# mjrgh/DCSExplorer

Hardware: AMD Instinct MI355X
Metric: bit_exact_int16_pcm_samples_per_sec (higher is better)
Workload: dtype int16; 1 GPU; survey3_65536; gpu_max_hw_queues=4, samples_per_frame=240, frames_per_wave=8, wavefronts_per_launch=8192, arithmetic=ADSP-2105 1.15 fixed point, 32-bit integer intermediates, partition=range over streams, no collective, scale=1, inflight=1, frames_per_chunk=all, full=False

## Files before the change

### dcsexplorer_amd/csrc/dcs_decode_chunk.inc.h

```cpp
    DCS_STAMP(1);

    struct { uint32_t job; uint32_t prevSlot, flags, nSrc, shiftXform; uint32_t firstSrc, prevJob, poolOff, bpl; } slot;
    uint32_t exportNext;
    uint4 pd0, pd1, phdr;
    uint2 pd2;
    uint32_t planHdr0 = 0, planHdr1 = 0, planType0 = 0, planType1 = 0;
    {
        uint4 *scratch = reinterpret_cast<uint4 *>(L.pool());
        static_assert(kHeadVec * 16 <= poolDwords(FPW) * 4, "the package head fits in the bit pool");
        if (lane < kHeadVec)
            scratch[lane] = phead0;
        if (kHeadLoads > 1 && lane + 64 < kHeadVec)
            scratch[lane + 64] = phead1;
        waveSync();
        const uint4 *sp5 = scratch + 5 * s;
        const uint4 s0 = sp5[0];
        pd0 = sp5[1]; pd1 = sp5[2];
        const uint4 d2v = sp5[3];
        pd2 = make_uint2(d2v.x, d2v.y);
        phdr = sp5[4];
        if constexpr (bandPlanInLds(FPW))
        {
            const unsigned char *bytes = reinterpret_cast<const unsigned char *>(sp5) + q;
            planType0 = bytes[36]; planType1 = bytes[44];
            planHdr0 = bytes[64]; planHdr1 = bytes[72];
        }
        waveSync();
        slot.job = s0.x;
        slot.prevSlot = s0.y & 0xFFu; slot.flags = (s0.y >> 8) & 0xFFu; slot.nSrc = (s0.y >> 16) & 0xFFu; slot.shiftXform = s0.y >> 24;
        slot.firstSrc = s0.z; slot.prevJob = s0.w;
        slot.poolOff = d2v.z & 0xFFFFu;
        slot.bpl = (d2v.z >> 16) & 0xFFu;
        const unsigned long long exportSlots = __ballot(lane < FPW && !(slot.flags & DCS_SLOT_EMPTY) && (slot.flags & DCS_SLOT_EXPORT) != 0);
        exportNext = static_cast<uint32_t>(__builtin_amdgcn_readlane(static_cast<int>(d2v.w), exportSlots != 0 ? static_cast<int>(__builtin_ctzll(exportSlots)) : 0));
    }

    if constexpr (bandPlanInLds(FPW))
    {
        const int fmt0 = static_cast<int>((pd0.z >> 16) & 0xFFu);
        if (__any(!(slot.flags & DCS_SLOT_EMPTY) && slot.nSrc != 0 && fmt0 >= DCS_FMT_94_T0))
        {
            uint2 *plan = reinterpret_cast<uint2 *>(L.plan());
            const uint2 *tmpl = reinterpret_cast<const uint2 *>(smem + planTableOffset(FPW));
            const bool type1 = fmt0 != DCS_FMT_94_T0;
            const uint32_t keyLim = type1 ? 16u : 17u;
            const uint32_t cls0 = !type1 ? DCS_B94_TYPE0 : q < 3 ? 0u : q < 6 ? 17u : 34u, cls1 = type1 ? 34u : DCS_B94_TYPE0;
            const uint32_t pre = (type1 && q < 3) ? (pd2.y >> (4 * q)) & 15u : 0u;
            plan[lane] = planBand94(L.tables(), tmpl, planHdr0, planType0, cls0, keyLim, q < 2 ? 7u + q : 16u, pre);
            plan[lane + 64] = planBand94(L.tables(), tmpl, planHdr1, planType1, cls1, keyLim, q == 7 ? 32u : 16u, 0u);
        }
    }

    const int firstXform = __builtin_amdgcn_readfirstlane(static_cast<int>(slot.shiftXform >> 4)) == DCS_XFORM_94 ? DCS_XFORM_94 : DCS_XFORM_93;
    if (PASS == 0 || firstXform != constsXform)
    {
        constsXform = firstXform;
        loadLaneConsts(a.tables, lane, constsXform, C);
    }
#pragma unroll
    for (int t = 0 ; t < kPoolPieces ; ++t)
    {
        const int i = lane * 4 + 256 * t;
        const bool in = i < imgDw;
        if (i < poolDwords(FPW))
            ldsWrite4(L.pool() + i, in ? pimg[t].x : 0u, in ? pimg[t].y : 0u, in ? pimg[t].z : 0u, in ? pimg[t].w : 0u);
    }

    const bool live = !(slot.flags & DCS_SLOT_EMPTY);
    struct { uint32_t firstSrc; int nSrc; int volShift; int xform; uint32_t prev; } job;
    job.firstSrc = slot.firstSrc; job.nSrc = slot.nSrc; job.volShift = slot.shiftXform & 15;
    job.xform = slot.shiftXform >> 4; job.prev = slot.prevJob;

    uint32_t err = 0;
    {
        uint32_t *pool = L.pool();
        const DcsLdsTables *T = L.tables();
        uint16_t *row = L.row(s);
        const uint32_t *blobW = reinterpret_cast<const uint32_t *>(a.blob);
        const uint32_t blobWords = static_cast<uint32_t>((a.blobLen + 3) >> 2);
        const int myNSrc = live ? job.nSrc : 0;

        auto unpackRound = [&](auto r0tag, const int r)
        {
            constexpr bool R0 = decltype(r0tag)::value;
            const bool has = r < myNSrc;
            const uint4 *sdp = reinterpret_cast<const uint4 *>(&a.srcs[has ? job.firstSrc + r : 0]);
            uint4 d0 = make_uint4(0, 0, 0, 0), d1 = d0;
            uint2 d2 = make_uint2(0, 0);
            uint2 sp = make_uint2(0, 0);
            const int bplSlot = slot.bpl;
            if (R0)
            {
                if (has) { d0 = pd0; d1 = pd1; d2 = pd2; sp = psplit; }
            }
            else if (has) { d0 = sdp[0]; d1 = sdp[1]; d2 = *reinterpret_cast<const uint2 *>(sdp + 2); }
            const uint64_t streamOff = static_cast<uint64_t>(d0.x) | (static_cast<uint64_t>(d0.y) << 32);
            const uint32_t mixMul = d0.z & 0xFFFFu;
            const int format = static_cast<int>((d0.z >> 16) & 0xFFu);
            const int hdrLen = has ? static_cast<int>(d0.z >> 24) : 16;
            const uint32_t bitOff = d0.w;
            const uint32_t nBits = d1.x & 0xFFFFu, hdrBits = d1.x >> 16;
            const int nBands = static_cast<int>((d2.y >> 16) & 0xFFu);
            const uint32_t flags = d2.y >> 24;
            const bool serial = R0 ? bplSlot == 0 : ((flags & DCS_IDX_SERIAL) != 0 || SUB == 1);

            Quarter Q;
            Q.t0 = d1.y; Q.t1 = d1.z; Q.t2 = d1.w; Q.t3 = d2.x;
            Q.preAdj = d2.y & 0xFFFFu;

            const uint64_t bitPos = (streamOff + 2 + static_cast<uint64_t>(hdrLen)) * 8 + bitOff;
            uint32_t off;
            bool fits;
            if (R0)
            {
                off = min(static_cast<uint32_t>(slot.poolOff), static_cast<uint32_t>(poolDwords(FPW) - 1));
                fits = true;
            }
            else
            {
                const uint32_t startDw = static_cast<uint32_t>(bitPos >> 5);
                const uint32_t nDw = (has && q == 0) ? dcsPoolDwords(streamOff, static_cast<uint32_t>(hdrLen), bitOff, nBits) : 0u;
                uint32_t incl = nDw;
#pragma unroll
                for (int d = 1 ; d < 64 ; d <<= 1)
                {
                    const uint32_t up = __shfl_up(incl, d);
                    if (lane >= d) incl += up;
                }
                const uint32_t offMine = incl - nDw;
                off = __shfl(offMine, s);
                const uint32_t nDwSlot = __shfl(nDw, s);
                fits = off + nDwSlot <= static_cast<uint32_t>(poolDwords(FPW));
                constexpr int kStageUnroll = FPW < 8 ? FPW : 8;
                for (int t0 = 0 ; t0 < FPW ; t0 += kStageUnroll)
                {
                    uint32_t v[kStageUnroll], dst[kStageUnroll];
                    bool any64 = false;
#pragma unroll
                    for (int u = 0 ; u < kStageUnroll ; ++u)
                    {
                        const uint32_t n = static_cast<uint32_t>(__builtin_amdgcn_readlane(static_cast<int>(nDw), t0 + u));
                        const uint32_t st = static_cast<uint32_t>(__builtin_amdgcn_readlane(static_cast<int>(startDw), t0 + u));
                        const uint32_t o = static_cast<uint32_t>(__builtin_amdgcn_readlane(static_cast<int>(offMine), t0 + u));
                        const bool room = o + n <= static_cast<uint32_t>(poolDwords(FPW));
                        const uint32_t w = st + static_cast<uint32_t>(lane);
                        const bool mine = room && static_cast<uint32_t>(lane) < n;
                        v[u] = (mine && w < blobWords) ? blobW[w] : 0u;
                        dst[u] = mine ? o + static_cast<uint32_t>(lane) : 0xFFFFFFFFu;
                        any64 = any64 || (room && n > 64);
                    }
#pragma unroll
                    for (int u = 0 ; u < kStageUnroll ; ++u)
                        if (dst[u] != 0xFFFFFFFFu)
                            pool[dst[u]] = __builtin_bswap32(v[u]);
                    if (any64)
                    {
                        for (int u = 0 ; u < kStageUnroll ; ++u)
                        {
                            const uint32_t n = static_cast<uint32_t>(__builtin_amdgcn_readlane(static_cast<int>(nDw), t0 + u));
                            const uint32_t st = static_cast<uint32_t>(__builtin_amdgcn_readlane(static_cast<int>(startDw), t0 + u));
                            const uint32_t o = static_cast<uint32_t>(__builtin_amdgcn_readlane(static_cast<int>(offMine), t0 + u));
                            if (o + n > static_cast<uint32_t>(poolDwords(FPW)))
                                continue;
                            for (uint32_t i = static_cast<uint32_t>(lane) + 64 ; i < n ; i += 64)
                            {
                                const uint32_t w = st + i;
                                pool[o + i] = w < blobWords ? __builtin_bswap32(blobW[w]) : 0u;
                            }
                        }
                    }
                }
            }

            if (R0) DCS_STAMP(2);
            if (R0)
            {
                Q.h0 = has ? phdr.x : 0u; Q.h1 = has ? phdr.y : 0u; Q.h2 = has ? phdr.z : 0u; Q.h3 = has ? phdr.w : 0u;
            }
            else
            {
                const uint32_t hw = static_cast<uint32_t>((streamOff + 2) >> 2);
                const uint32_t sh = static_cast<uint32_t>((streamOff + 2) & 3);
                uint32_t hdrW[5];
#pragma unroll
                for (int i = 0 ; i < 5 ; ++i)
                    hdrW[i] = (has && hw + i < blobWords) ? blobW[hw + i] : 0u;
                Q.h0 = __builtin_amdgcn_alignbyte(hdrW[1], hdrW[0], sh);
                Q.h1 = __builtin_amdgcn_alignbyte(hdrW[2], hdrW[1], sh);
                Q.h2 = __builtin_amdgcn_alignbyte(hdrW[3], hdrW[2], sh);
                Q.h3 = __builtin_amdgcn_alignbyte(hdrW[4], hdrW[3], sh);
                if (hdrLen == 1)
                {
                    Q.h0 &= 0xFFu; Q.h1 = Q.h2 = Q.h3 = 0;
                }
            }
            waveSync();

            if (R0) DCS_STAMP(3);
            const bool ok = has && fits && unpacker;
            if (has && !fits && q == 0)
                err |= DCS_FRAME_FATAL | DCS_FRAME_STOP;
            if (has && q == 0)
                err |= flags >> 4;
            uint32_t relBits = hdrBits;
            Q.bandBase = 0;
            Q.outIdx = 1;
            Q.prv = 0; Q.prvDelta = 0;
            Q.subType = (format == DCS_FMT_93B_T1) ? 0 : 2;
            Q.reuse = false; Q.first = true;
            Q.midEnd = Q.midStart = Q.midStraddle = false;
            if (serial)
                Q.nb = (q == 0) ? nBands : 0;
            else
            {
                const int nb16 = min(nBands, 16);
                if (R0)
                {
                    const bool f93a = format == DCS_FMT_93A_T1;
                    const int nbEnd = f93a ? min(nBands, 18) : nb16;
                    const int myBase = (sp.x & 0x8000u) ? nbEnd
                                     : static_cast<int>(sp.y >> 28) + ((f93a && (sp.y & (DCS_SPLIT_BASE16 << 16)) != 0) ? 16 : 0);
                    const int nextBase = __shfl(myBase, lane + FPW);
                    Q.bandBase = myBase;
                    Q.nb = max((q == SUB - 1 ? nbEnd : nextBase) - myBase, 0);
                    if (SUB == 16)
                    {
                        const bool mid = format >= DCS_FMT_94_T0 && q == SUB - 1 && myBase == 15 && (sp.y & (DCS_SPLIT_MID15 << 16)) != 0;
                        const bool nextMid = __shfl(static_cast<int>(mid), lane + FPW) != 0;
                        Q.midStart = mid;
                        Q.midStraddle = mid && (sp.y & (DCS_MID15_STRADDLE << 16)) != 0;
                        Q.midEnd = q == SUB - 2 && nextMid;
                        if (Q.midEnd)
                            Q.nb = 16 - myBase;
                    }
                }
                else
                {
                    const int bpl = max((nb16 + SUB - 1) / SUB, 1);
                    if (format == DCS_FMT_93A_T1)
                    {
                        Q.bandBase = min(q * bpl, nb16);
                        Q.nb = min(max(nb16 - Q.bandBase, 0), bpl);
                    }
                    else
                    {
                        Q.bandBase = dcsLaneFirstBand(format, q, bpl, nb16);
                        Q.nb = (q == SUB - 1 ? nb16 : dcsLaneFirstBand(format, q + 1, bpl, nb16)) - Q.bandBase;
                    }
                }
                if (q != 0 && Q.nb != 0)
                {
                    if (!R0)
                        sp = reinterpret_cast<const uint2 *>(sdp)[5 + Q.bandBase - 1];
                    const uint32_t sp0 = sp.x, sp1 = sp.y;
                    relBits = sp0 & 0x7FFFu;
                    Q.prv = sp0 >> 16;
                    Q.prvDelta = sp1 & 0xFFFFu;
                    const uint32_t st = sp1 >> 16;
                    Q.outIdx = static_cast<int>(st & 0x1FFu);
                    Q.subType = static_cast<int>((st >> 9) & 3u);
                    Q.reuse = (st & 0x800u) != 0;
                    Q.first = false;
                }
            }
            const uint32_t inPool = static_cast<uint32_t>(bitPos & 31) + relBits;
            const uint32_t *brAt = pool + (ok ? off + (inPool >> 5) : 0u);
            const int brBit = static_cast<int>(inPool & 31);

            if (R0) DCS_STAMP(12);
            const bool is94 = ok && format >= DCS_FMT_94_T0;
            const bool is93a = ok && format == DCS_FMT_93A_T1 && Q.nb != 0 && !(Q.bandBase != 0 && Q.reuse);
            const bool is93 = ok && format < DCS_FMT_93A_T1;
            if (__any(is94))
            {
                BR94 br;
                br.init(brAt, brBit);
                const uint32_t planAt = (R0 && bandPlanInLds(FPW))
                    ? static_cast<uint32_t>(reinterpret_cast<uintptr_t>((LdsBytePtr)L.plan())) + static_cast<uint32_t>(Q.bandBase * FPW + s) * kPlanRecBytes
                    : 0u;
                err |= unpack94<R0, BR94, SUB>(T, row, br, Q, format, mixMul, is94, stamp, planAt);
            }
            BR93 br;
            br.init(brAt, brBit);
            if (__any(is93))
                err |= unpack93<R0, BR93>(T, row, br, Q, format, mixMul, is93, stamp);
            if (is93a)
            {
                constexpr bool kSpreadTail = SUB == 16 && !R0;
                const int end = Q.bandBase + Q.nb;
                const int end2 = (!R0 && SUB != 16 && end >= 16 && nBands > 16) ? nBands : end;
                const int prv0 = Q.bandBase == 0 ? 0x1A : sx16(Q.prv), out0 = Q.bandBase == 0 ? 0 : Q.outIdx;
                const int hb0 = static_cast<int>(Q.h0 & 0xFFu);
                if (pairTableInLds(FPW))
                    err |= unpack93a<R0, BR93>(T, row, br, hb0, mixMul, reinterpret_cast<const uint16_t *>(smem + ldsBytes(FPW) - 4096),
                                         Q.bandBase, end2, prv0, out0);
                else
                    err |= unpack93a<R0, BR93>(T, row, br, hb0, mixMul, a.tables->pair93a, Q.bandBase, end2, prv0, out0);
                if (kSpreadTail && pairTableInLds(FPW) && q < 2 && 16 + q < nBands)
                {
                    const uint32_t r0 = q == 0 ? Q.t0 : Q.t2, r1 = q == 0 ? Q.t1 : Q.t3;
                    if (!((r1 >> 16) & 0x800u))
                    {
                        const uint32_t inPool2 = static_cast<uint32_t>(bitPos & 31) + (r0 & 0xFFFFu);
                        BR93 br2;
                        br2.init(pool + off + (inPool2 >> 5), static_cast<int>(inPool2 & 31));
                        err |= unpack93a<R0, BR93>(T, row, br2, hb0, mixMul, reinterpret_cast<const uint16_t *>(smem + ldsBytes(FPW) - 4096),
                                             16 + q, 17 + q, sx16(r0 >> 16), static_cast<int>((r1 >> 16) & 0x1FFu));
                    }
                }
            }
            waveSync();
        };

        {
            if (__any(myNSrc > 0))
                unpackRound(std::true_type{}, 0);
            for (int r = 1 ; __any(r < myNSrc) ; ++r)
                unpackRound(std::false_type{}, r);
        }

        DCS_STAMP(4);
        if (__any(err != 0))
        {
#pragma unroll
            for (int m = FPW ; m < 64 ; m <<= 1)
                err |= __shfl_xor(err, m);
        }
        if (live && q == 0)
        {
            if (job.xform == DCS_XFORM_93)
// ... 194 lines not shown
```

### dcsexplorer_amd/csrc/dcs_kernels.hip.h

```cpp
#pragma once
#include <hip/hip_runtime.h>
#include <type_traits>
#include <cstddef>
#include "dcs_common.h"

namespace dcsk {

struct Stamper
{
#ifdef DCS_STAMPS
    unsigned long long *p;
#ifdef DCS_STAMPS_REALTIME
    __device__ __forceinline__ void operator()(int k) const { if (p != nullptr) p[k] = __builtin_amdgcn_s_memrealtime(); }
#else
    __device__ __forceinline__ void operator()(int k) const { if (p != nullptr) p[k] = __builtin_amdgcn_s_memtime(); }
#endif
#else
    __device__ __forceinline__ void operator()(int) const { }
#endif
};
#define DCS_STAMP(k) stamp(k)

__device__ __forceinline__ unsigned long long handoffWord(uint32_t epoch, uint32_t who, uint32_t payload)
{
// ... 133 lines not shown
    __device__ __forceinline__ uint32_t get(int n) { const uint32_t v = peek(n); skip(n); return v; }
    __device__ __forceinline__ uint32_t bitAddr() const { return bp + 1u; }
    __device__ __forceinline__ void initAt(uint32_t bits) { bp = bits - 1u; }
    __device__ __forceinline__ uint32_t mark() const { return bitAddr(); }
    __device__ __forceinline__ void initAtMark(uint32_t m) { initAt(m); }
};

template <class BR>
__device__ __forceinline__ int readVlc(BR &br, const uint16_t *fast, const uint16_t *trie)
{
    uint32_t e = fast[br.peek(8)];
    if (e & 0x8000)
    {
        br.skip(static_cast<int>((e >> 8) & 0xF));
        return static_cast<int>(e & 0xFF);
    }
    br.skip(8);
    uint32_t w = br.cur();
    int n = 0;
    do
    {
        e = trie[e + (w >> 31)];
        w <<= 1;
        ++n;
    }
    while (!(e & 0x8000) && n < 24);
    br.skip(n);
    return static_cast<int>(e & 0xFF);
}

template <int FPW>
struct Lds
{
    unsigned char *tab;
    unsigned char *base;
    unsigned char *poolBase;
    __device__ __forceinline__ const DcsLdsTables *tables() const { return reinterpret_cast<const DcsLdsTables *>(tab); }
    __device__ __forceinline__ uint16_t *row(int s) const { return reinterpret_cast<uint16_t *>(base + s * kRowBytes); }
    __device__ __forceinline__ uint16_t *tails() const { return reinterpret_cast<uint16_t *>(base + FPW * kRowBytes); }
    __device__ __forceinline__ uint32_t *pool() const { return reinterpret_cast<uint32_t *>(poolBase); }
    __device__ __forceinline__ unsigned char *plan() const { return base + FPW * kRowBytes + (FPW + 1) * 32; }
};

struct Quarter
{
    uint32_t h0, h1, h2, h3;
    uint32_t t0, t1, t2, t3;
    int bandBase;
    int nb;
    int outIdx;
    uint32_t preAdj;
    uint32_t prv, prvDelta;
    int subType;
    bool reuse, first;
    bool midEnd, midStart, midStraddle;
};

__device__ __forceinline__ int byteOf(uint32_t w0, uint32_t w1, uint32_t w2, uint32_t w3, int b)
{
    const int i = b >> 2;
    const uint32_t lo = (i & 1) ? w1 : w0, hi = (i & 1) ? w3 : w2;
    const uint32_t w = (i & 2) ? hi : lo;
    return static_cast<int>((w >> (8 * (b & 3))) & 0xFFu);
}

__device__ __forceinline__ int mul24(int a, int b)
{
    int r;
    asm("v_mul_i32_i24 %0, %1, %2" : "=v"(r) : "v"(a), "v"(b));
    return r;
}

template <bool FIRST>
__device__ __forceinline__ void mixAdd(uint16_t *cell, int scaledProduct, uint32_t mixMul)
{
    uint32_t t, acc;
    asm("v_mul_i32_i24_sdwa %0, sext(%1), %2 dst_sel:DWORD dst_unused:UNUSED_PAD src0_sel:WORD_0 src1_sel:DWORD"
        : "=v"(t) : "v"(scaledProduct), "v"(mixMul));
    asm("v_add_u32_sdwa %0, %1, %2 dst_sel:DWORD dst_unused:UNUSED_PAD src0_sel:DWORD src1_sel:WORD_0"
        : "=v"(acc) : "v"(t), "v"(scaledProduct));
    if (!FIRST)
        acc += static_cast<uint32_t>(*cell) << 16;
    *cell = static_cast<uint16_t>(acc >> 16);
}
typedef uint16_t __attribute__((address_space(3))) *LdsWordPtr;
template <bool FIRST>
__device__ __forceinline__ void mixAddAt(uint32_t cellAddr, int scaledProduct, uint32_t mixMul)
{
    const LdsWordPtr cell = reinterpret_cast<LdsWordPtr>(static_cast<uintptr_t>(cellAddr));
    uint32_t t, acc;
    asm("v_mul_i32_i24_sdwa %0, sext(%1), %2 dst_sel:DWORD dst_unused:UNUSED_PAD src0_sel:WORD_0 src1_sel:DWORD"
        : "=v"(t) : "v"(scaledProduct), "v"(mixMul));
    asm("v_add_u32_sdwa %0, %1, %2 dst_sel:DWORD dst_unused:UNUSED_PAD src0_sel:DWORD src1_sel:WORD_0"
        : "=v"(acc) : "v"(t), "v"(scaledProduct));
    if (!FIRST)
        acc += static_cast<uint32_t>(*cell) << 16;
    *cell = static_cast<uint16_t>(acc >> 16);
}
template <bool FIRST>
__device__ __forceinline__ uint32_t mixAddCarry(uint16_t *cell, int scaledProduct, uint32_t mixMul, uint32_t addLow)
{
    uint32_t t, acc;
    asm("v_mul_i32_i24_sdwa %0, sext(%1), %2 dst_sel:DWORD dst_unused:UNUSED_PAD src0_sel:WORD_0 src1_sel:DWORD"
        : "=v"(t) : "v"(scaledProduct), "v"(mixMul));
    asm("v_add_u32_sdwa %0, %1, %2 dst_sel:DWORD dst_unused:UNUSED_PAD src0_sel:DWORD src1_sel:WORD_0"
        : "=v"(acc) : "v"(t), "v"(addLow));
    if (!FIRST)
        acc += static_cast<uint32_t>(*cell) << 16;
    *cell = static_cast<uint16_t>(acc >> 16);
    return acc;
}
template <bool FIRST>
__device__ __forceinline__ uint32_t mixAddCarryAt(uint32_t cellAddr, int scaledProduct, uint32_t mixMul, uint32_t addLow)
{
    const LdsWordPtr cell = reinterpret_cast<LdsWordPtr>(static_cast<uintptr_t>(cellAddr));
    uint32_t t, acc;
    asm("v_mul_i32_i24_sdwa %0, sext(%1), %2 dst_sel:DWORD dst_unused:UNUSED_PAD src0_sel:WORD_0 src1_sel:DWORD"
        : "=v"(t) : "v"(scaledProduct), "v"(mixMul));
    asm("v_add_u32_sdwa %0, %1, %2 dst_sel:DWORD dst_unused:UNUSED_PAD src0_sel:DWORD src1_sel:WORD_0"
        : "=v"(acc) : "v"(t), "v"(addLow));
    if (!FIRST)
        acc += static_cast<uint32_t>(*cell) << 16;
    *cell = static_cast<uint16_t>(acc >> 16);
    return acc;
}
__device__ __forceinline__ int mulLowWord(uint32_t x, int y)
{
    int r;
    asm("v_mul_i32_i24_sdwa %0, sext(%1), %2 dst_sel:DWORD dst_unused:UNUSED_PAD src0_sel:WORD_0 src1_sel:DWORD" : "=v"(r) : "v"(x), "v"(y));
    return r;
}
__device__ __forceinline__ void mixSub(uint16_t *cell, int scaledProduct, uint32_t mixMul)
{
    const uint32_t s = static_cast<uint32_t>(scaledProduct) & 0xFFFFu;
    const uint32_t c = (s + static_cast<uint32_t>(__mul24(sx16(s), static_cast<int>(mixMul)))) >> 16;
    *cell = static_cast<uint16_t>(*cell - c);
}

__device__ __forceinline__ uint32_t scaleFactor(const DcsLdsTables *T, int code)
{
    return T->scale64[code & 63];
}

__device__ __forceinline__ void dcFixup(uint16_t *row, uint32_t saved1)
{
    const int delta = sat16(sx16(row[1]) - sx16(saved1));
    row[0] = static_cast<uint16_t>(sat16(delta + sx16(row[0])));
    row[1] = static_cast<uint16_t>(saved1);
}

constexpr int kDummyWord = 256;

typedef uint8_t __attribute__((address_space(3))) *LdsBytePtr;
__device__ __forceinline__ uint2 planBand94(const DcsLdsTables *T, const uint2 *tmpl, uint32_t hdrByte, uint32_t typeByte,
                                            uint32_t cls, uint32_t keyLim, uint32_t count0, uint32_t pre)
{
    const uint32_t strided = (hdrByte >> 6) & 1u;
    const uint2 t = tmpl[min(typeByte, keyLim) + (strided * 72u + cls)];
    const uint32_t scale = scaleFactor(T, static_cast<int>(hdrByte + pre + ((t.x >> 16) & 0x7Fu)));
    const uint32_t book = static_cast<uint32_t>(reinterpret_cast<uintptr_t>((LdsWordPtr)reinterpret_cast<const uint16_t *>(T))) + (t.x & 0xFFFFu);
    const uint32_t span = static_cast<uint32_t>(__mul24(static_cast<int>(count0 >> strided), static_cast<int>(t.x >> 24)));
    return make_uint2(book | (scale << 16), t.y | (span << 24));
}

template <bool FIRST, class BR, int SUB>
__device__ uint32_t unpack94(const DcsLdsTables *T, uint16_t *row, BR &br, const Quarter &Q,
                             int format, uint32_t mixMul, bool has, const Stamper &stamp, uint32_t planAt = 0)
{
    constexpr bool kPlan = FIRST && SUB == 8;
    constexpr uint32_t kPlanBandBytes = kPlanRecBytes * 8;
    const bool type1 = format != DCS_FMT_94_T0;
    uint32_t err = 0;
    int nb = has ? Q.nb : 0;
    const int b1 = Q.bandBase + nb;
    const int before = Q.bandBase <= 0 ? 0 : Q.bandBase == 1 ? 7 : 15 + 16 * (Q.bandBase - 2);
    const int upTo = b1 <= 0 ? 0 : b1 == 1 ? 7 : b1 >= 16 ? 255 : 15 + 16 * (b1 - 2);
    const int midAdvance = 16 - (Q.midStraddle ? 1 + static_cast<int>((Q.h3 >> 30) & 1u) : 0);
    int outIdx = min(Q.outIdx, 256 - ((SUB == 16 && Q.midStart) ? midAdvance : upTo - before));
    bool valid = true;
    const bool owner = has && Q.bandBase == 0;
    const uint32_t saved1 = (owner && !FIRST) ? row[1] : 0u;

    stamp(8);
    int k = 0;
    uint32_t planEnd = planAt + kPlanBandBytes * static_cast<uint32_t>(nb);
    const int keyLim = type1 ? 16 : 17;
    uint32_t cell = static_cast<uint32_t>(reinterpret_cast<uintptr_t>((LdsWordPtr)row)) + 2u * static_cast<uint32_t>(outIdx);
    uint32_t cellEnd = cell;
    uint32_t cellStart = cell;
    uint32_t startBits = 0;
    const uint16_t *book = T->cb94;
    int shPeek = 0, shIdx = 0, scale = 0;
    uint32_t incSh = 1;
    uint32_t valOff = 0, valWidth = 8;
    for (int round = 0 ; ; ++round)
    {
        if (SUB == 16 && Q.midEnd && cell > cellEnd)
            cellEnd = cell;
        if (cell > cellEnd)
        {
            cell -= 1u << incSh;
            if (valid)
            {
                BR r2;
                if (kPlan)
                    r2.initAtMark(startBits);
                else
                    r2.initAt(startBits);
                uint32_t c2 = cellStart;
                while (c2 + (1u << incSh) < cellEnd)
                {
                    const uint32_t e = book[r2.cur() >> shIdx];
                    r2.skip(static_cast<int>((e >> 8) & 0x1F));
                    const uint32_t step = e >> 13;
                    if (step == 1)
                        mixSub((uint16_t *)reinterpret_cast<LdsWordPtr>(static_cast<uintptr_t>(c2)),
                               mul24(static_cast<int>(static_cast<int8_t>(e & 0xFF)), scale), mixMul);
                    c2 += step << incSh;
                }
            }
            valid = false; err |= DCS_FRAME_STOP;
            cellEnd = cell;
        }
        const bool start = cell == cellEnd && (kPlan ? planAt < planEnd : k < nb);
        if (!__any(start || cell < cellEnd))
            break;
        if constexpr (kPlan)
        {
            if (start)
            {
                const LdsBytePtr rec = reinterpret_cast<LdsBytePtr>(static_cast<uintptr_t>(planAt));
                planAt += kPlanBandBytes;
                const uint32_t bookAt = *reinterpret_cast<LdsWordPtr>(rec);
                const uint32_t recScale = *reinterpret_cast<LdsWordPtr>(rec + 2);
                const uint32_t recOff = rec[5], recWidth = rec[6], span = rec[7];
                shIdx = rec[4];
                book = (const uint16_t *)reinterpret_cast<LdsWordPtr>(static_cast<uintptr_t>(bookAt));
                valOff = recOff;
                valWidth = recWidth;
                incSh = __builtin_amdgcn_ubfe(recOff, 5u, 2u);
                if (recOff > 0x7Fu)
                {
                    err |= DCS_FRAME_FATAL | DCS_FRAME_STOP;
                    planEnd = 0;
                }
                scale = valid ? static_cast<int>(recScale) : 0;
                cellEnd = cell + span;
                cell = recWidth > 0x7Fu ? cellEnd : cell;
                cellStart = cell;
                startBits = br.mark();
            }
        }
        else if (start)
        {
            const int band = Q.bandBase + k;
            ++k;
            const int hb = byteOf(Q.h0, Q.h1, Q.h2, Q.h3, band) & 0x7F;
            const int code0 = byteOf(Q.t0, Q.t1, Q.t2, Q.t3, band);
            const int cls = band < 3 ? 0 : band < 6 ? 17 : 34;
            const int key = min(code0, keyLim) + (type1 ? cls : DCS_B94_TYPE0);
            const uint32_t e = T->band94[key];
            const int count0 = band < 2 ? 7 + band : band == 15 ? 32 : 16;
            const uint32_t strided = (static_cast<uint32_t>(hb) >> 6) & 1u;
            const uint32_t count = static_cast<uint32_t>(count0) >> strided;
            incSh = 1u + strided;
            const int pre = (type1 && band < 3) ? static_cast<int>((Q.preAdj >> (4 * band)) & 15u) : 0;
            scale = static_cast<int>(scaleFactor(T, hb + pre + static_cast<int>(e >> 25)));
            book = reinterpret_cast<const uint16_t *>(T) + (e & 0x7FFu);
            shPeek = static_cast<int>((e >> 11) & 31u);
            shIdx = static_cast<int>((e >> 16) & 31u);
            const bool isRaw = (e & DCS_B94_RAW) != 0;
            valOff = isRaw ? static_cast<uint32_t>(shPeek) : 0u;
            valWidth = isRaw ? 32u - static_cast<uint32_t>(shPeek) : 8u;
            const bool zeroBand = (e & DCS_B94_ZERO) != 0, fatal = (e & DCS_B94_FATAL) != 0;
            uint32_t i = (e & (DCS_B94_ZERO | DCS_B94_FATAL)) == 0 ? count : 0u;
            if (SUB == 16 && band == 15 && i != 0)
            {
                if (Q.midEnd) i = count - (count >> 1);
                if (Q.midStart) i = (count >> 1) - (Q.midStraddle ? 1u : 0u);
            }
            cell += zeroBand ? 2u * count : 0u;
            if (fatal)
            {
                err |= DCS_FRAME_FATAL | DCS_FRAME_STOP;
                nb = 0;
            }
            if (!valid)
                scale = 0;
            cellStart = cell;
            cellEnd = cell + (i << incSh);
            startBits = br.bitAddr();
        }

        if (round == 0) stamp(9);
        const uint32_t roundLen = round == 0 ? 7u : round == 1 ? 9u : 16u;
        const uint32_t roundEnd = min(cellEnd, cell + (roundLen << incSh));
        if (cell < roundEnd)
        {
            do
            {
                const uint32_t ahead = br.prefetch();
                const uint32_t w = br.cur();
                const uint32_t e = book[w >> shIdx];
                const int v = __builtin_amdgcn_sbfe(__builtin_amdgcn_perm(w, e, 0x07060100u), valOff, valWidth);
                const uint32_t step = e >> 13;
                br.skipTight((e >> 8) & 0x1Fu, ahead);
// ... 646 lines not shown
    stageB<true, 4, 3>(x, C.k + DCS_K94_TWB, R);
    DCS_PACE_STEP(2);
    stageB<true, 2, 2>(x, C.k + DCS_K94_TWB + 2, R);
    stageB<true, 1, 1>(x, C.k + DCS_K94_TWB + 6, R);
    if (__any(P.shiftPair != 0))
    {
#pragma unroll
        for (int r = 0 ; r < 16 ; ++r)
            x[r] = pkAshr(x[r], P.shiftPair);
    }
}

template <int STEPS>
__device__ __forceinline__ void transform93x4(const PassLane &P, const TwA &W, const LaneConsts &C, BflyRegs &R, uint32_t (&x)[16])
{
    const int l = P.l;
    uint32_t *S = P.rowC;
#pragma unroll
    for (int r = 0 ; r < 8 ; ++r)
    {
        const int p = 16 * r + l;
        const uint32_t A = P.rowC[p];
        const uint32_t B = P.rowC[(128 - p) & 127];
        const uint32_t Sm = pkAdd(A, B), Df = pkSub(A, B);
        x[r] = __builtin_amdgcn_perm(Df, Sm, 0x07060100u);
        x[r + 8] = __builtin_amdgcn_perm(Sm, Df, 0x07060100u);
        if (p == 0)
        {
            x[0] = A; x[8] = A;
        }
    }
    DCS_XSTAMP(8);
    DCS_PACE_STEP(0);
    stageA<false, 4, 3>(x, W, R);
    stageA<false, 2, 2>(x, W, R);
    stageA<false, 1, 1>(x, W, R);
    DCS_XSTAMP(9);
    waveSync();
    uint32_t y[16];
#pragma unroll
    for (int h = 0 ; h < 2 ; ++h)
    {
#pragma unroll
        for (int r = 0 ; r < 8 ; ++r)
            S[swzPos(r, l)] = x[8 * h + r];
        waveSync();
        if ((l >> 3) == h)
        {
#pragma unroll
            for (int c = 0 ; c < 4 ; ++c)
            {
                const uint4 v = ldsRead4(S + swzQuad(l & 7, c));
                y[4 * c] = v.x; y[4 * c + 1] = v.y; y[4 * c + 2] = v.z; y[4 * c + 3] = v.w;
            }
        }
        waveSync();
    }
#pragma unroll
    for (int r = 0 ; r < 16 ; ++r)
        x[r] = y[r];
    DCS_XSTAMP(10);
    DCS_PACE_STEP(1);
    stageB<false, 8, 4>(x, C.k + DCS_K93_TWB, R);
    stageB<false, 4, 3>(x, C.k + DCS_K93_TWB + 1, R);
    DCS_PACE_STEP(2);
    stageB<false, 2, 2>(x, C.k + DCS_K93_TWB + 3, R);
    stageB<false, 1, 1>(x, C.k + DCS_K93_TWB + 7, R);
    DCS_XSTAMP(11);
    if (__any(P.shiftPair != 0))
    {
#pragma unroll
        for (int r = 0 ; r < 16 ; ++r)
            x[r] = pkAshr(x[r], P.shiftPair);
    }
}

#ifndef DCS_CPW2_SCHED
#define DCS_CPW2_SCHED 1
#endif
struct PaceSchedule { int entry; bool steps; int levels; };
__host__ __device__ constexpr PaceSchedule paceSchedule(int cpw, int pass)
{
    if (cpw == 1)
        return { 3, true, kPaceSteps };
#if DCS_CPW2_SCHED == 0
    return pass == 0 ? PaceSchedule{ 3, false, kPaceSteps } : PaceSchedule{ 3, true, 2 | (1 << 2) | (0 << 4) };
#elif DCS_CPW2_SCHED == 1
    return pass == 0 ? PaceSchedule{ 3, false, kPaceSteps } : PaceSchedule{ 2, true, 1 | (1 << 2) | (0 << 4) };
#elif DCS_CPW2_SCHED == 2
    return pass == 0 ? PaceSchedule{ 3, true, 3 | (3 << 2) | (2 << 4) } : PaceSchedule{ 2, true, 1 | (1 << 2) | (0 << 4) };
#else
    return pass == 0 ? PaceSchedule{ 3, true, 3 | (2 << 2) | (2 << 4) } : PaceSchedule{ 1, true, 1 | (0 << 2) | (0 << 4) };
#endif
}

template <int FPW, int CPW = 1>
#ifndef DCS_MIN_WAVES
#define DCS_MIN_WAVES 4
#endif
__global__ void __launch_bounds__(64 * kWavesPerBlock, DCS_MIN_WAVES)
dcsDecodeKernel(uint8_t *kPackages, const DcsDevTables *kTables, uint32_t kNChunks, uint32_t kFlags, uint32_t kEpoch, uint32_t kNJobs,
                int16_t *kPcm, unsigned long long *kHandoff, uint32_t *kErr, int16_t *kTailsOut,
                const uint8_t *kBlob, uint64_t kBlobLen, const DcsSrcDesc *kSrcs, const int16_t *kTailsIn, unsigned long long *kDebug)
{
    DcsKernelArgs a;
    a.blob = kBlob; a.blobLen = kBlobLen; a.srcs = kSrcs; a.packages = kPackages; a.nChunks = kNChunks; a.nJobs = kNJobs;
    a.pcm = kPcm; a.err = kErr; a.tailsIn = kTailsIn; a.tailsOut = kTailsOut; a.tables = kTables; a.debug = kDebug;
    a.handoff = kHandoff; a.epoch = kEpoch; a.flags = kFlags;
    extern __shared__ __attribute__((aligned(16))) unsigned char smem[];
    const int wave = static_cast<int>(threadIdx.x) >> 6;
    const int lane = static_cast<int>(threadIdx.x) & 63;
    constexpr int kPoolBytes = poolDwords(FPW) * 4, kTileBytes = waveTileBytes(FPW);
    static_assert(kPoolBytes % 16 == 0 && kWavesPerBlock * kTileBytes >= 8192, "LDS layout");
    const Lds<FPW> L{ smem, smem + DCS_LDS_DECODE_BYTES + kWavesPerBlock * kPoolBytes + wave * kTileBytes,
                      smem + DCS_LDS_DECODE_BYTES + wave * kPoolBytes };
    uint32_t blk = blockIdx.x;
    if (a.flags & DCS_BATCH_XCD_RANGES)
        blk = (blk & 7u) * (gridDim.x >> 3) + (blk >> 3);
    static_assert(CPW == 1 || CPW == 2, "one or two chunks per wavefront");
    const uint32_t wv = blk * kWavesPerBlock + static_cast<uint32_t>(wave);
    const uint32_t nFirst = CPW == 2 ? (a.nChunks + 1u) >> 1 : a.nChunks;
    auto stamperOf = [&](uint32_t chunk, bool valid)
    {
#ifdef DCS_STAMPS
        return Stamper{ (lane == 0 && a.debug != nullptr && valid) ? a.debug + static_cast<size_t>(chunk) * 16 : nullptr };
#else
        return Stamper{};
#endif
    };
    {
        const Stamper stamp = stamperOf(wv, wv < nFirst);
        DCS_STAMP(0);
    }
    const bool pacedLaunch = (a.flags & DCS_BATCH_PACED) != 0;
    const bool paced = pacedLaunch && blockIdx.x + ((a.flags >> DCS_BATCH_CUS8_SHIFT) & 0xFFu) * 32u >= gridDim.x;
    if (pacedLaunch) __builtin_amdgcn_s_setprio(3);
    constexpr int SUB = subLanes(FPW);
#ifndef DCS_DIRECT_MAX_FPW
#define DCS_DIRECT_MAX_FPW 4
#endif
    using BR94 = typename std::conditional<(FPW <= DCS_DIRECT_MAX_FPW), DirectReader, BitReader>::type;
    using BR93 = DirectReader;
    static_assert(SUB * FPW == 64 && SUB <= 16, "every lane unpacks; a frame has at most 16 split lanes");
    const int s = lane % FPW;
    const int q = lane / FPW;
    const bool unpacker = q < SUB;

    const uint32_t layout = (a.flags >> DCS_BATCH_IMG_SHIFT) & DCS_BATCH_IMG_MASK;
    const int imgDw = static_cast<int>(dcsPkgImgDw(layout));
    const bool split4 = (layout & DCS_PKG_SPLIT4) != 0;
    const uint32_t offPool = split4 ? dcsPkgOffPool(FPW, DCS_PKG_SPLIT4) : dcsPkgOffPool(FPW, 0);
    constexpr int kHeadVec = FPW * 5, kHeadLoads = (kHeadVec + 63) / 64;
    static_assert(kHeadLoads <= 2, "package head: two 16-byte loads per lane at most");
    uint4 phead0, phead1 = make_uint4(0, 0, 0, 0);
    uint2 psplit;
    constexpr int kPoolPieces = (poolDwords(FPW) + 255) / 256;
    uint4 pimg[kPoolPieces];
    {
        const uint32_t chunk = wv;
        const bool valid = wv < nFirst;
#include "dcs_request_package.inc.h"
    }
    TwA W;
    loadTwA(a.tables, W);

    {
        constexpr int kTableVec = DCS_LDS_DECODE_BYTES / 16;
        static_assert(kTableVec <= 64 * kWavesPerBlock, "one piece of the tables per thread");
        const uint4 piece = reinterpret_cast<const uint4 *>(&a.tables->lds)[min(static_cast<int>(threadIdx.x), kTableVec - 1)];
        const bool stagePairs = pairTableInLds(FPW) && (a.flags & DCS_BATCH_HAS_93A_T1);
        uint4 pairPiece = make_uint4(0, 0, 0, 0);
        if (stagePairs)
            pairPiece = reinterpret_cast<const uint4 *>(a.tables->pair93a)[threadIdx.x];
        uint4 *tile = reinterpret_cast<uint4 *>(L.base);
        if constexpr (bandPlanInLds(FPW))
        {
            constexpr int kPlanVec = DCS_PLAN94_BYTES / 16;
            const uint4 planPiece = reinterpret_cast<const uint4 *>(a.tables->plan94)[min(static_cast<int>(threadIdx.x), kPlanVec - 1)];
            for (int i = lane ; i < FPW * kRowBytes / 16 ; i += 64)
                tile[i] = make_uint4(0, 0, 0, 0);
            if (static_cast<int>(threadIdx.x) < kPlanVec)
                reinterpret_cast<uint4 *>(smem + planTableOffset(FPW))[threadIdx.x] = planPiece;
        }
#ifndef DCS_CLEAR_FIRST_MAX_FPW
#define DCS_CLEAR_FIRST_MAX_FPW 8
#endif
        constexpr bool kClearFirst = FPW <= DCS_CLEAR_FIRST_MAX_FPW;
        if (kClearFirst && !bandPlanInLds(FPW))
            for (int i = lane ; i < FPW * kRowBytes / 16 ; i += 64)
                tile[i] = make_uint4(0, 0, 0, 0);
        if (static_cast<int>(threadIdx.x) < kTableVec)
            reinterpret_cast<uint4 *>(smem)[threadIdx.x] = piece;
        if (stagePairs)
            reinterpret_cast<uint4 *>(smem + ldsBytes(FPW) - 4096)[threadIdx.x] = pairPiece;
        if (!kClearFirst)
            for (int i = lane ; i < FPW * kRowBytes / 16 ; i += 64)
                tile[i] = make_uint4(0, 0, 0, 0);
    }
    __syncthreads();
    if (wv >= nFirst)
        return;

    int constsXform = -1;
    LaneConsts C;
    if constexpr (CPW == 1)
    {
        constexpr int PASS = 0;
        constexpr PaceSchedule kPace = paceSchedule(CPW, PASS);
        const uint32_t chunk = wv;
        const Stamper stamp = stamperOf(chunk, true);
#include "dcs_decode_chunk.inc.h"
    }
    else
    {
        auto decodeChunk = [&](const uint32_t chunk, auto passTag)
        {
            constexpr int PASS = decltype(passTag)::value;
            constexpr PaceSchedule kPace = paceSchedule(CPW, PASS);
            const Stamper stamp = stamperOf(chunk, true);
#include "dcs_decode_chunk.inc.h"
        };
        decodeChunk(wv, std::integral_constant<int, 0>{});
        const uint32_t second = wv + nFirst;
        if (second < a.nChunks)
        {
            {
                const Stamper stamp0 = stamperOf(second, true);
                stamp0(0);
            }
            constexpr PaceSchedule kPace = paceSchedule(CPW, 1);
            if (paced && kPace.entry != 3) __builtin_amdgcn_s_setprio(kPace.entry);
            {
                const uint32_t chunk = second;
                const bool valid = true;
#include "dcs_request_package.inc.h"
            }
            uint4 *tile = reinterpret_cast<uint4 *>(L.base);
            for (int i = lane ; i < FPW * kRowBytes / 16 ; i += 64)
                tile[i] = make_uint4(0, 0, 0, 0);
            waveSync();
            decodeChunk(second, std::integral_constant<int, 1>{});
        }
    }
}

}
```

### dcsexplorer_amd/csrc/dcs_request_package.inc.h

```cpp
        const uint8_t *pkg = a.packages + (valid ? static_cast<size_t>(chunk) * (offPool + static_cast<uint32_t>(imgDw) * 4u) : 0);
        static_assert(sizeof(DcsSlot) == 32 && offsetof(DcsSlot, runStartDw) == 16 && offsetof(DcsSlot, nextJob) == 24 && DCS_PKG_SLOT_BYTES == 80, "DcsSlot / package layout");
        phead0 = reinterpret_cast<const uint4 *>(pkg)[min(lane, kHeadVec - 1)];
        if (kHeadLoads > 1)
            phead1 = reinterpret_cast<const uint4 *>(pkg)[min(lane + 64, kHeadVec - 1)];
        if (split4)
        {
            const uint32_t raw = *reinterpret_cast<const uint32_t *>(pkg + dcsPkgOffSplit(FPW) + static_cast<uint32_t>(lane) * 4u);
            psplit = make_uint2(raw & 0xFFFFu, raw & 0xFFFF0000u);
        }
        else
            psplit = *reinterpret_cast<const uint2 *>(pkg + dcsPkgOffSplit(FPW) + static_cast<uint32_t>(lane) * 8u);
#pragma unroll
        for (int t = 0 ; t < kPoolPieces ; ++t)
        {
            const int i = min(lane * 4 + 256 * t, imgDw - 4);
            pimg[t] = *reinterpret_cast<const uint4 *>(pkg + offPool + i * 4);
        }
```

Measured before the change: 513.9 billion samples/s.

## Load package head and bit pool straight into LDS with global_load_lds

When there is one chunk per wave and the band plan sits in LDS, the package head and bit-pool image are fetched with global_load_lds directly into LDS. This replaces the path of loading into VGPRs and then writing to LDS, which frees registers and removes the LDS write pass. Only the tail past the image is zero-filled. Tile clears use inline-asm ds_write, and explicit s_waitcnt barriers order the DMA against the clears. A lean R0 path also drops the has-guards and split masking to cut VALU work, at the cost of correctness relying on empty slots being harmless.

Result: no change. 515.4 billion samples/s, median of 2 (+0.3%).

```diff
diff --git a/dcsexplorer_amd/csrc/dcs_decode_chunk.inc.h b/dcsexplorer_amd/csrc/dcs_decode_chunk.inc.h
--- a/dcsexplorer_amd/csrc/dcs_decode_chunk.inc.h
+++ b/dcsexplorer_amd/csrc/dcs_decode_chunk.inc.h
@@ -5,14 +5,18 @@
     uint4 pd0, pd1, phdr;
     uint2 pd2;
     uint32_t planHdr0 = 0, planHdr1 = 0, planType0 = 0, planType1 = 0;
-    {
-        uint4 *scratch = reinterpret_cast<uint4 *>(L.pool());
+    const uint2 split = (kLeanR0 && split4) ? make_uint2(psplit.x & 0xFFFFu, psplit.x & 0xFFFF0000u) : psplit;
+    {
+        uint4 *scratch = reinterpret_cast<uint4 *>(kPkgDma ? L.plan() : reinterpret_cast<unsigned char *>(L.pool()));
         static_assert(kHeadVec * 16 <= poolDwords(FPW) * 4, "the package head fits in the bit pool");
-        if (lane < kHeadVec)
-            scratch[lane] = phead0;
-        if (kHeadLoads > 1 && lane + 64 < kHeadVec)
-            scratch[lane + 64] = phead1;
-        waveSync();
+        if constexpr (!kPkgDma)
+        {
+            if (lane < kHeadVec)
+                scratch[lane] = phead0;
+            if (kHeadLoads > 1 && lane + 64 < kHeadVec)
+                scratch[lane + 64] = phead1;
+            waveSync();
+        }
         const uint4 *sp5 = scratch + 5 * s;
         const uint4 s0 = sp5[0];
         pd0 = sp5[1]; pd1 = sp5[2];
@@ -57,13 +61,29 @@
         constsXform = firstXform;
         loadLaneConsts(a.tables, lane, constsXform, C);
     }
-#pragma unroll
-    for (int t = 0 ; t < kPoolPieces ; ++t)
-    {
-        const int i = lane * 4 + 256 * t;
-        const bool in = i < imgDw;
-        if (i < poolDwords(FPW))
-            ldsWrite4(L.pool() + i, in ? pimg[t].x : 0u, in ? pimg[t].y : 0u, in ? pimg[t].z : 0u, in ? pimg[t].w : 0u);
+    if constexpr (kPkgDma)
+    {
+        if (imgDw < poolDwords(FPW))
+        {
+#pragma unroll
+            for (int t = 0 ; t < kPoolPieces ; ++t)
+            {
+                const int i = lane * 4 + 256 * t;
+                if (i >= imgDw && i < poolDwords(FPW))
+                    ldsWrite4(L.pool() + i, 0u, 0u, 0u, 0u);
+            }
+        }
+    }
+    else
+    {
+#pragma unroll
+        for (int t = 0 ; t < kPoolPieces ; ++t)
+        {
+            const int i = lane * 4 + 256 * t;
+            const bool in = i < imgDw;
+            if (i < poolDwords(FPW))
+                ldsWrite4(L.pool() + i, in ? pimg[t].x : 0u, in ? pimg[t].y : 0u, in ? pimg[t].z : 0u, in ? pimg[t].w : 0u);
+        }
     }
 
     const bool live = !(slot.flags & DCS_SLOT_EMPTY);
@@ -91,7 +111,7 @@
             const int bplSlot = slot.bpl;
             if (R0)
             {
-                if (has) { d0 = pd0; d1 = pd1; d2 = pd2; sp = psplit; }
+                if (kLeanR0 || has) { d0 = pd0; d1 = pd1; d2 = pd2; sp = split; }
             }
             else if (has) { d0 = sdp[0]; d1 = sdp[1]; d2 = *reinterpret_cast<const uint2 *>(sdp + 2); }
             const uint64_t streamOff = static_cast<uint64_t>(d0.x) | (static_cast<uint64_t>(d0.y) << 32);
@@ -175,7 +195,8 @@
             if (R0) DCS_STAMP(2);
             if (R0)
             {
-                Q.h0 = has ? phdr.x : 0u; Q.h1 = has ? phdr.y : 0u; Q.h2 = has ? phdr.z : 0u; Q.h3 = has ? phdr.w : 0u;
+                const bool hdr = kLeanR0 || has;
+                Q.h0 = hdr ? phdr.x : 0u; Q.h1 = hdr ? phdr.y : 0u; Q.h2 = hdr ? phdr.z : 0u; Q.h3 = hdr ? phdr.w : 0u;
             }
             else
             {
diff --git a/dcsexplorer_amd/csrc/dcs_kernels.hip.h b/dcsexplorer_amd/csrc/dcs_kernels.hip.h
--- a/dcsexplorer_amd/csrc/dcs_kernels.hip.h
+++ b/dcsexplorer_amd/csrc/dcs_kernels.hip.h
@@ -309,6 +309,23 @@
 constexpr int kDummyWord = 256;
 
 typedef uint8_t __attribute__((address_space(3))) *LdsBytePtr;
+typedef const void __attribute__((address_space(1))) *GlobalPiecePtr;
+typedef void __attribute__((address_space(3))) *LdsPiecePtr;
+#ifndef DCS_PKG_DMA
+#define DCS_PKG_DMA 1
+#endif
+typedef uint32_t __attribute__((ext_vector_type(4))) Dwords4;
+template <bool UNSEEN>
+__device__ __forceinline__ void ldsClear16(uint4 *p)
+{
+    if constexpr (UNSEEN)
+    {
+        const Dwords4 zero = { 0u, 0u, 0u, 0u };
+        asm volatile("ds_write_b128 %0, %1" : : "v"(static_cast<uint32_t>(reinterpret_cast<uintptr_t>((LdsBytePtr)p))), "v"(zero) : "memory");
+    }
+    else
+        *p = make_uint4(0, 0, 0, 0);
+}
 __device__ __forceinline__ uint2 planBand94(const DcsLdsTables *T, const uint2 *tmpl, uint32_t hdrByte, uint32_t typeByte,
                                             uint32_t cls, uint32_t keyLim, uint32_t count0, uint32_t pre)
 {
@@ -1261,6 +1278,8 @@
     const uint32_t offPool = split4 ? dcsPkgOffPool(FPW, DCS_PKG_SPLIT4) : dcsPkgOffPool(FPW, 0);
     constexpr int kHeadVec = FPW * 5, kHeadLoads = (kHeadVec + 63) / 64;
     static_assert(kHeadLoads <= 2, "package head: two 16-byte loads per lane at most");
+    constexpr bool kPkgDma = DCS_PKG_DMA != 0 && bandPlanInLds(FPW) && CPW == 1;
+    constexpr bool kLeanR0 = CPW == 1;
     uint4 phead0, phead1 = make_uint4(0, 0, 0, 0);
     uint2 psplit;
     constexpr int kPoolPieces = (poolDwords(FPW) + 255) / 256;
@@ -1287,7 +1306,7 @@
             constexpr int kPlanVec = DCS_PLAN94_BYTES / 16;
             const uint4 planPiece = reinterpret_cast<const uint4 *>(a.tables->plan94)[min(static_cast<int>(threadIdx.x), kPlanVec - 1)];
             for (int i = lane ; i < FPW * kRowBytes / 16 ; i += 64)
-                tile[i] = make_uint4(0, 0, 0, 0);
+                ldsClear16<kPkgDma>(tile + i);
             if (static_cast<int>(threadIdx.x) < kPlanVec)
                 reinterpret_cast<uint4 *>(smem + planTableOffset(FPW))[threadIdx.x] = planPiece;
         }
@@ -1306,6 +1325,8 @@
             for (int i = lane ; i < FPW * kRowBytes / 16 ; i += 64)
                 tile[i] = make_uint4(0, 0, 0, 0);
     }
+    if constexpr (kPkgDma)
+        asm volatile("s_waitcnt vmcnt(0) lgkmcnt(0)" ::: "memory");
     __syncthreads();
     if (wv >= nFirst)
         return;
@@ -1339,6 +1360,8 @@
             }
             constexpr PaceSchedule kPace = paceSchedule(CPW, 1);
             if (paced && kPace.entry != 3) __builtin_amdgcn_s_setprio(kPace.entry);
+            if constexpr (kPkgDma)
+                asm volatile("s_waitcnt lgkmcnt(0)" ::: "memory");
             {
                 const uint32_t chunk = second;
                 const bool valid = true;
@@ -1346,7 +1369,9 @@
             }
             uint4 *tile = reinterpret_cast<uint4 *>(L.base);
             for (int i = lane ; i < FPW * kRowBytes / 16 ; i += 64)
-                tile[i] = make_uint4(0, 0, 0, 0);
+                ldsClear16<kPkgDma>(tile + i);
+            if constexpr (kPkgDma)
+                asm volatile("s_waitcnt vmcnt(0) lgkmcnt(0)" ::: "memory");
             waveSync();
             decodeChunk(second, std::integral_constant<int, 1>{});
         }
diff --git a/dcsexplorer_amd/csrc/dcs_request_package.inc.h b/dcsexplorer_amd/csrc/dcs_request_package.inc.h
--- a/dcsexplorer_amd/csrc/dcs_request_package.inc.h
+++ b/dcsexplorer_amd/csrc/dcs_request_package.inc.h
@@ -1,18 +1,39 @@
         const uint8_t *pkg = a.packages + (valid ? static_cast<size_t>(chunk) * (offPool + static_cast<uint32_t>(imgDw) * 4u) : 0);
         static_assert(sizeof(DcsSlot) == 32 && offsetof(DcsSlot, runStartDw) == 16 && offsetof(DcsSlot, nextJob) == 24 && DCS_PKG_SLOT_BYTES == 80, "DcsSlot / package layout");
-        phead0 = reinterpret_cast<const uint4 *>(pkg)[min(lane, kHeadVec - 1)];
-        if (kHeadLoads > 1)
-            phead1 = reinterpret_cast<const uint4 *>(pkg)[min(lane + 64, kHeadVec - 1)];
+        if constexpr (kPkgDma)
+        {
+            static_assert(kHeadLoads == 1 && 64 * 16 <= planBytes(FPW), "one 16-byte piece per lane fills the plan area at most");
+            __builtin_amdgcn_global_load_lds((GlobalPiecePtr)(pkg + min(lane, kHeadVec - 1) * 16),
+                                             (LdsPiecePtr)L.plan(), 16, 0, 0);
+        }
+        else
+        {
+            phead0 = reinterpret_cast<const uint4 *>(pkg)[min(lane, kHeadVec - 1)];
+            if (kHeadLoads > 1)
+                phead1 = reinterpret_cast<const uint4 *>(pkg)[min(lane + 64, kHeadVec - 1)];
+        }
         if (split4)
         {
             const uint32_t raw = *reinterpret_cast<const uint32_t *>(pkg + dcsPkgOffSplit(FPW) + static_cast<uint32_t>(lane) * 4u);
-            psplit = make_uint2(raw & 0xFFFFu, raw & 0xFFFF0000u);
+            if constexpr (kLeanR0)
+                psplit.x = raw;
+            else
+                psplit = make_uint2(raw & 0xFFFFu, raw & 0xFFFF0000u);
         }
         else
             psplit = *reinterpret_cast<const uint2 *>(pkg + dcsPkgOffSplit(FPW) + static_cast<uint32_t>(lane) * 8u);
 #pragma unroll
         for (int t = 0 ; t < kPoolPieces ; ++t)
         {
-            const int i = min(lane * 4 + 256 * t, imgDw - 4);
-            pimg[t] = *reinterpret_cast<const uint4 *>(pkg + offPool + i * 4);
+            if constexpr (kPkgDma)
+            {
+                const int i = lane * 4 + 256 * t;
+                if (i < min(imgDw, poolDwords(FPW)))
+                    __builtin_amdgcn_global_load_lds((GlobalPiecePtr)(pkg + offPool + i * 4), (LdsPiecePtr)(L.pool() + 256 * t), 16, 0, 0);
+            }
+            else
+            {
+                const int i = min(lane * 4 + 256 * t, imgDw - 4);
+                pimg[t] = *reinterpret_cast<const uint4 *>(pkg + offPool + i * 4);
+            }
         }
```
